# lazytiger/pbrt-rs

Hardware: AMD Instinct MI355X
Metric: Mrays/s (higher is better)
Workload: dtype f32

## Files before the change

pbrt-rs_amd/csrc/render.hip:

```cpp
#include <hip/hip_runtime.h>
#include "abi_guard.h"

#include <algorithm>
#include <chrono>
#include <cstdio>
#include <cstdlib>
#include <cstring>
#include <string>
#include <thread>
#include <vector>

#include "scene.h"
#include "trace.h"
#include "wavefront.h"

using namespace pb;

extern "C" int pbrt_hip_render_device(PbrtHipScene* s, const PbrtCamera* camera, const PbrtRenderParams* params,
                                      float* d_film, PbrtRenderStats* stats) try {
    if (!s || !camera || !params || !d_film) return PBRT_HIP_ERR_INVALID;
    PB_ENTER(s->ctx);
    HIP_TRY(s->ctx, hipSetDevice(s->ctx->device));
    return wavefront_render(s, *camera, *params, d_film, stats);
}
// ... 622 lines not shown
        if (stats) *stats = local;
        return PBRT_HIP_OK;
    }
    const int n_pix = (int)origins.size() * kTile * kTile;
    int64_t valid_pixels = 0;
    for (const int2& o : origins)
        valid_pixels += (int64_t)(std::min(o.x + kTile, rp.x1) - o.x) * (std::min(o.y + kTile, rp.y1) - o.y);
    if (li_mode) valid_pixels = li->n;
    if (export_mode) rp.spp_per_pass = rp.spp;
    int spp_pass = rp.spp_per_pass > 0 ? rp.spp_per_pass : 0;
    if (spp_pass == 0) {
        size_t free_b = 0, total_b = 0;
        HIP_TRY(ctx, hipMemGetInfo(&free_b, &total_b));
        for (const auto& b : ctx->block_cache)
            if (!b.in_use) free_b += b.bytes;
        const int64_t per_path = 400 + (rp.integrator != PBRT_INTEGRATOR_PATH ? 24 + 48ll * std::max(1, rp.max_depth) : 0);
        const int64_t target_paths = std::max<int64_t>(1ll << 20, std::min<int64_t>(1ll << 28, (int64_t)(free_b / 2) / per_path));
        spp_pass = (int)std::max<int64_t>(1, std::min<int64_t>(rp.spp, target_paths / n_pix));
    }
    spp_pass = std::min(spp_pass, rp.spp);
    if (export_mode && spp_pass != rp.spp) return invalid("camera rays: too many samples for one pass");
    const size_t N = (size_t)n_pix * spp_pass;
    if (N * 4 >= (1ull << 32)) return invalid("too many concurrent paths for 32-bit queue entries; lower spp_per_pass");

    DevBuf buf(ctx);
    bool ok = true;
    PathState ps;
    ps.n_paths = N;
    ps.two_level = s->d.bvh.instanced ? 1 : 0;
    ps.ray = buf.alloc<float4>(N * 6, &ok);
    ps.hit = buf.alloc<float4>(N * 6, &ok);
    ps.rng = buf.alloc<uint64_t>(N, &ok);
    ps.L = buf.alloc<float4>(N, &ok);
    ps.beta = buf.alloc<float4>(N, &ok);
    ps.nee_a = buf.alloc<float4>(N, &ok);
    ps.nee_f = buf.alloc<float4>(N, &ok);
    ps.nee_b = buf.alloc<float4>(N, &ok);
    ps.nee_light = buf.alloc<int>(N, &ok);
    ps.pfilm = buf.alloc<float2>(N, &ok);
    Queues q[2];
    for (int k = 0; k < 2; ++k) {
        q[k].trace = buf.alloc<uint32_t>(N * 3, &ok);
        q[k].shade = buf.alloc<uint32_t>(N, &ok);
        q[k].counts64 = buf.alloc<unsigned long long>(2, &ok);
        q[k].keys = nullptr;
        for (int a = 0; a < 3; ++a) {
            const float lo = s->d.bvh.root_min[a], hi = s->d.bvh.root_max[a];
            q[k].key_lo[a] = lo;
            q[k].key_inv[a] = hi > lo ? 1.0f / (hi - lo) : 0.0f;
        }
    }
    if (rp.ray_order < 0 || rp.ray_order > 1) return invalid("ray_order must be 0 (Morton order from the second bounce on) or 1 (queue order)");
    const bool sort_rays = rp.ray_order == 0 && rp.integrator == PBRT_INTEGRATOR_PATH;
    constexpr int sort_from = 2;
// ... 3 lines not shown
    if (sort_rays) {
        sort_keys[0] = buf.alloc<uint32_t>(N * 3, &ok);
        sort_keys[1] = buf.alloc<uint32_t>(N * 3, &ok);
        sort_vals = buf.alloc<uint32_t>(N * 3, &ok);
        if (pb::sort_pairs_u32(st, nullptr, &sort_tmp_bytes, sort_keys[0], sort_keys[1], sort_vals, sort_vals, N * 3, kSortKeyBits) != 0)
            return invalid("rocPRIM radix sort: size query failed");
        sort_tmp = buf.alloc<char>(sort_tmp_bytes, &ok);
    }
    const bool use_wide = s->has_wide && ctx->count_traversal != 1 && ctx->traversal == PBRT_TRAVERSAL_AUTO;
    const bool stackless = ctx->traversal == PBRT_TRAVERSAL_STACKLESS;
    if (stackless && !stackless_applies(s)) return PBRT_HIP_ERR_INVALID;
    uint32_t* special_list = use_wide ? buf.alloc<uint32_t>(N * 3, &ok) : nullptr;
    if (rp.shade_order < 0 || rp.shade_order > 2) return invalid("shade_order must be 0 (queue order), 1 (by material inside blocks) or 2 (sorted queue)");
    const bool sort_shade = rp.shade_order == 2 && rp.integrator == PBRT_INTEGRATOR_PATH;
    const bool bin_shade = rp.shade_order == 1 && rp.integrator == PBRT_INTEGRATOR_PATH;
    uint32_t *shade_keys[2] = {nullptr, nullptr}, *shade_sorted = nullptr;
    void* shade_tmp = nullptr;
    size_t shade_tmp_bytes = 0;
    if (sort_shade) {
        shade_keys[0] = buf.alloc<uint32_t>(N, &ok);
        shade_keys[1] = buf.alloc<uint32_t>(N, &ok);
        shade_sorted = buf.alloc<uint32_t>(N, &ok);
        if (pb::sort_pairs_u32(st, nullptr, &shade_tmp_bytes, shade_keys[0], shade_keys[1], shade_sorted, shade_sorted, N, 3) != 0)
            return invalid("rocPRIM radix sort: size query failed");
        shade_tmp = buf.alloc<char>(shade_tmp_bytes, &ok);
    }
    DirectState ds{};
    std::vector<int> prefix(s->d.n_lights + 1, 0);
    for (int i = 0; i < s->d.n_lights; ++i)
        prefix[i + 1] = prefix[i] + (tabulated ? round_count(s->light_samples[i]) : s->light_samples[i]);
    SamplerParams smp{};
    smp.kind = rp.sampler;
    smp.n_dims = rp.sampler_dims;
    smp.nx = rp.sampler_x;
    smp.ny = rp.sampler_y;
    smp.jitter = rp.sampler_jitter;
    ps.samp = buf.alloc<int>(N, &ok);
    if (rp.sampler == PBRT_SAMPLER_HALTON) {
// ... 285 lines not shown
            if (direct)
{
                dim3 sg((n_shade + 255) / 256), sb(256);
                if (rp.integrator == PBRT_INTEGRATOR_DIRECT && s->glossy)
                    hipLaunchKernelGGL((k_shade_direct<PBRT_INTEGRATOR_DIRECT, true>), sg, sb, 0, st, sc, ps, ds, q[cur], q[nxt], pp, tiles, n_shade);
                else if (rp.integrator == PBRT_INTEGRATOR_DIRECT)
                    hipLaunchKernelGGL((k_shade_direct<PBRT_INTEGRATOR_DIRECT, false>), sg, sb, 0, st, sc, ps, ds, q[cur], q[nxt], pp, tiles, n_shade);
                else if (rp.integrator == PBRT_INTEGRATOR_WHITTED && s->glossy)
                    hipLaunchKernelGGL((k_shade_direct<PBRT_INTEGRATOR_WHITTED, true>), sg, sb, 0, st, sc, ps, ds, q[cur], q[nxt], pp, tiles, n_shade);
                else if (rp.integrator == PBRT_INTEGRATOR_WHITTED)
                    hipLaunchKernelGGL((k_shade_direct<PBRT_INTEGRATOR_WHITTED, false>), sg, sb, 0, st, sc, ps, ds, q[cur], q[nxt], pp, tiles, n_shade);
                else
                    hipLaunchKernelGGL((k_shade_direct<PBRT_INTEGRATOR_AO, false>), sg, sb, 0, st, sc, ps, ds, q[cur], q[nxt], pp, tiles, n_shade);
            }
            else {
                Queues qin = q[cur];
                if (sort_shade && wavefront >= 1 && n_shade >= (1u << 10)) {
                    hipLaunchKernelGGL(k_shade_sort_keys, dim3((n_shade + 255) / 256), dim3(256), 0, st, sc, ps, q[cur].shade, n_shade,
                                       pp.max_depth, shade_keys[0]);
                    size_t tb = shade_tmp_bytes;
                    if (pb::sort_pairs_u32(st, shade_tmp, &tb, shade_keys[0], shade_keys[1], q[cur].shade, shade_sorted, n_shade, 3) != 0 &&
                        rc == PBRT_HIP_OK) {
                        ctx->last_error = "rocPRIM radix sort failed";
                        rc = PBRT_HIP_ERR_DEVICE;
                    }
                    qin.shade = shade_sorted;
                }
                const dim3 sg((n_shade + 255) / 256), sb(256);
                if (bin_shade && wavefront >= 1 && s->glossy)
                    hipLaunchKernelGGL((k_shade<true, true>), sg, sb, 0, st, sc, ps, qin, q[nxt], pp, tiles, n_shade);
                else if (bin_shade && wavefront >= 1)
                    hipLaunchKernelGGL((k_shade<true, false>), sg, sb, 0, st, sc, ps, qin, q[nxt], pp, tiles, n_shade);
                else if (s->glossy)
                    hipLaunchKernelGGL((k_shade<false, true>), sg, sb, 0, st, sc, ps, qin, q[nxt], pp, tiles, n_shade);
                else
                    hipLaunchKernelGGL((k_shade<false, false>), sg, sb, 0, st, sc, ps, qin, q[nxt], pp, tiles, n_shade);
            }
            RENDER_TRY(hipGetLastError());
            RENDER_TRY(hipMemcpyAsync(ctx->h_counts, q[nxt].counts64, sizeof(counts), hipMemcpyDeviceToHost, st));
            RENDER_TRY(hipEventRecord(ctx->ev_sync, st));
            if (rc == PBRT_HIP_OK) {
                hipError_t qe;
                const auto spin_start = std::chrono::steady_clock::now();
                uint32_t polls = 0;
                while ((qe = hipEventQuery(ctx->ev_sync)) == hipErrorNotReady) {
                    if ((++polls & 0xfffu) == 0) {
                        const double waited = std::chrono::duration<double>(std::chrono::steady_clock::now() - spin_start).count();
                        if (waited > ctx->wavefront_deadline_s) {
                            ctx->last_error = "a wavefront did not finish within the deadline (hung kernel?)";
                            ctx->lost = true;
                            rc = PBRT_HIP_ERR_DEVICE;
                            break;
                        }
                        if (waited > 0.05) std::this_thread::yield();
                    }
                }
                if (rc == PBRT_HIP_OK) RENDER_TRY(qe);
            }
            counts[0] = ctx->h_counts[0];
            counts[1] = ctx->h_counts[1];
            if (n_trace > 0 && rc == PBRT_HIP_OK) {
                float ms = 0.0f;
                RENDER_TRY(hipEventElapsedTime(&ms, e_t0, e_t1));
                local.trace_ms += ms;
                local.trace_launches += 1;
                if (ctx->trace_log)
                    std::fprintf(stderr, "[pbrt_hip] k_trace: %u rays %.3f ms (%.0f Mrays/s)\n", n_trace, ms, n_trace / ms * 1e-3);
                ctx->trace_ms += ms;
                ctx->trace_launches += 1;
            }
            {
                uint64_t n_rays = counts[0] & 0xffffffffull, n_shadow = counts[0] >> 32;
                local.rays_closest += n_rays - n_shadow;
                local.rays_shadow += n_shadow;
                counts[0] = n_rays;
            }
            (void)first;
            first = false;
            wavefront += 1;
            cur = nxt;
        }
        if (li_mode) {
// ... 56 lines not shown
```

pbrt-rs_amd/csrc/wf_direct.h:

```cpp
#pragma once
#include "wf_path.h"

namespace pb {

struct DirectState {
    int* stage;
    float4* ld_acc;
    float4* frames;
    int light_strategy;
    int mode;
    int ao_samples;
    int ao_cos_sample;
};

#ifndef PB_DIRECT_WAVES
#define PB_DIRECT_WAVES 2
#endif
template <int MODE, bool GLOSSY>
__global__ void __launch_bounds__(256, (GLOSSY && MODE == PBRT_INTEGRATOR_DIRECT) ? 1 : PB_DIRECT_WAVES) k_shade_direct(ShadeConsts sc, PathState ps, DirectState ds, Queues qin,
                                                        Queues qout, PassParams pp, TileList tiles, uint32_t n_in) {
    uint32_t i = blockIdx.x * blockDim.x + threadIdx.x;
    bool active = i < n_in;
    uint32_t p = active ? qin.shade[i] : 0u;
    bool emit_cont = false, emit_mis = false, emit_shadow = false, mis_bool = false;
// ... 187 lines not shown
                    pick_pdf = 1.0f / nl;
                }
                float ul0, ul1, us0, us1;
                if (sample_all && tabulated && !fallback) {
                    int k = stage - sc.light_sample_prefix[light_num];
                    int first = (sm.arr & 0x7fff) - 2 * sc.n_lights + 2 * light_num;
                    samp_array_2d(pp, sm, first, k, &ul0, &ul1);
                    samp_array_2d(pp, sm, first + 1, k, &us0, &us1);
                } else {
                    samp_2d(pp, sm, &ul0, &ul1);
                    samp_2d(pp, sm, &us0, &us1);
                }
                int nee_flags;
                if (GLOSSY) {
                    NsBsdf nsb = ns_bsdf(sc.materials[sf.material]);
                    nee_flags = estimate_direct_emit(sc, ps, p, sf, fr, nsb.n > 0, nsb, light_num, ul0, ul1, us0, us1, pick_pdf, T);
                } else {
                    bool matte = (mat.type == PBRT_MAT_MATTE) && !is_black(kd);
                    nee_flags = estimate_direct_emit(sc, ps, p, sf, fr, matte, MatteBsdf{kd}, light_num, ul0, ul1, us0, us1, pick_pdf, T);
                }
                stage += 1;
                if (nee_flags) {
                    flags |= nee_flags & 0xff;
                    emit_shadow = (nee_flags & PF_NEE_SHADOW) != 0;
                    emit_mis = (nee_flags & PF_NEE_MIS) != 0;
                    mis_bool = (nee_flags & NEE_MIS_BOOL) != 0;
                    break;
                }
                close_light_if_done(stage);
                continue;
            }
            bool branched = false;
            if ((stage == total || stage == total + 1) && depth + 1 < pp.max_depth && mode != PBRT_INTEGRATOR_AO) {
                if (!surface_ready) load_surface();
// ... 67 lines not shown
```

pbrt-rs_amd/csrc/wf_lights.h:

```cpp
#pragma once
#include "wf_microfacet.h"

namespace pb {

PB_DEV V3 sphere_through(V3 v) {
    return V3{1.0f * v.x + 0.0f * v.y + 0.0f * v.z, 0.0f * v.x + 1.0f * v.y + 0.0f * v.z, 0.0f * v.x + 0.0f * v.y + 1.0f * v.z};
}
PB_DEV float sphere_area(float radius) { return (360.0f * (kPi / 180.0f)) * radius * (radius - (-radius)); }
PB_DEV void sphere_light_sample(float cx, float cy, float cz, float radius, const Surf& sf, float u0, float u1, V3* p_o,
                                V3* err_o, V3* n_o, float* pdf_o) {
    V3 pc = V3{1.0f * 0.0f + 0.0f * 0.0f + 0.0f * 0.0f + cx, 0.0f * 0.0f + 1.0f * 0.0f + 0.0f * 0.0f + cy,
               0.0f * 0.0f + 0.0f * 0.0f + 1.0f * 0.0f + cz};
    V3 p_origin = offset_ray_origin(sf.p, sf.p_error, sf.n, pc - sf.p);
    if (len2(p_origin - pc) <= radius * radius) {
        float z = 1.0f - 2.0f * u0;
        float rr = __builtin_sqrtf(fmaxr(1.0f - z * z, 0.0f));
        float sp, cp;
        det_sincos(2.0f * kPi * u1, &sp, &cp);
        V3 obj = V3{rr * cp, rr * sp, z} * radius;
        V3 n = normalize(sphere_through(obj));
        obj = obj * (radius / length(obj));
        V3 oe = vabs(obj) * kGamma5;
        const float g3 = kGamma3;
        V3 p = V3{1.0f * obj.x + 0.0f * obj.y + 0.0f * obj.z + cx, 0.0f * obj.x + 1.0f * obj.y + 0.0f * obj.z + cy,
// ... 216 lines not shown
    for (int j = 0; j < n; ++j) sum += func[j];
    float avg = sum / (float)(128 * n);
    float min_contrib = avg > 0.0f ? 0.001f * avg : 1.0f;
    for (int j = 0; j < n; ++j) func[j] = fmaxr(func[j], min_contrib);
    cdf[0] = 0.0f;
    for (int j = 1; j < n + 1; ++j) cdf[j] = cdf[j - 1] + func[j - 1] / (float)n;
    float func_int = cdf[n];
    if (func_int == 0.0f) {
        for (int j = 1; j < n + 1; ++j) cdf[j] = (float)j / (float)n;
    } else {
        for (int j = 1; j < n + 1; ++j) cdf[j] /= func_int;
    }
    func[2 * n + 1] = func_int;
}

template <class Bsdf>
PB_DEV int estimate_direct_emit(const ShadeConsts& sc, const PathState& ps, uint32_t p, const Surf& sf, const Frame& fr,
                                bool nonspecular, const Bsdf& bsdf, int light_num, float ul0, float ul1, float us0, float us1,
                                float pick_pdf, V3 beta) {
    if (!nonspecular) return 0;
    V3 wo = sf.wo;
    DevLight lt = sc.lights[light_num];
    V3 wi, li, p1, p1_err, p1_n;
    float light_pdf;
    light_sample_li(sc, sf, lt, ul0, ul1, &wi, &light_pdf, &li, &p1, &p1_err, &p1_n);
    int nee_flags = 0;
    V3 A = V3{0.0f, 0.0f, 0.0f};
    if (light_pdf > 0.0f && !is_black(li)) {
        V3 f;
        float scattering_pdf;
        bsdf_f_pdf(bsdf, fr, wo, wi, &f, &scattering_pdf);
        f = f * absdot(wi, fr.ns);
        if (!is_black(f)) {
            V3 origin = offset_ray_origin(sf.p, sf.p_error, sf.n, p1 - sf.p);
            V3 target = offset_ray_origin(p1, p1_err, p1_n, origin - p1);
            V3 d = target - origin;
            store_ray(ps, p, RS_SHADOW, origin, d, 1.0f - kShadowEpsilon);
            if (lt.delta) {
                A = mulv(li, f) / light_pdf;
            } else {
                float weight = power_heuristic1(light_pdf, scattering_pdf);
                A = mulv(li, f) * weight / light_pdf;
            }
            nee_flags |= PF_NEE_SHADOW;
        }
    }
    V3 wi2;
    float spdf = 0.0f;
    bool ok = false;
    V3 f2 = V3{0.0f, 0.0f, 0.0f};
    if (!lt.delta) f2 = bsdf_sample_f(bsdf, fr, wo, us0, us1, &wi2, &spdf, &ok);
    if (ok) f2 = f2 * absdot(wi2, fr.ns);
// ... 40 lines not shown
            if (ph < 0.0f) ph = ph + 2.0f * kPi;
            float st = det_sin(theta);
            if (st == 0.0f) {
                lpdf = 0.0f;
            } else {
                int iu = (int)(ph * kInv2Pi * 2.0f);
                iu = iu < 0 ? 0 : (iu > 1 ? 1 : iu);
                int iv = (int)(theta * kInvPi * 2.0f);
                iv = iv < 0 ? 0 : (iv > 1 ? 1 : iv);
                lpdf = sc.env_cond_func[iv][iu] / sc.env_marg_int / (2.0f * kPi * kPi * st);
            }
        }
        if (lpdf != 0.0f) {
            float weight = power_heuristic1(spdf, lpdf);
            V3 o2 = offset_ray_origin(sf.p, sf.p_error, sf.n, wi2);
            store_ray(ps, p, RS_MIS, o2, wi2, kInf);
            ps.nee_f[p] = make_float4(f2.x, f2.y, f2.z, weight);
            nee_flags |= PF_NEE_MIS;
            if (sc.mis_bool && lt.type != PBRT_LIGHT_DIFFUSE_AREA) nee_flags |= NEE_MIS_BOOL;
        }
    }
    if (nee_flags) {
        ps.nee_a[p] = make_float4(A.x, A.y, A.z, pick_pdf);
        ps.nee_b[p] = make_float4(beta.x, beta.y, beta.z, spdf);
        ps.nee_light[p] = light_num;
    }
    return nee_flags;
}

PB_DEV V3 estimate_direct_resolve(const ShadeConsts& sc, const PathState& ps, uint32_t p, int flags, float* pick_pdf,
                                  V3* beta_at_vertex) {
    float4 na = ps.nee_a[p], nf = ps.nee_f[p], nb = ps.nee_b[p];
    int light_id = ps.nee_light[p];
    V3 ld = V3{0.0f, 0.0f, 0.0f};
    if (flags & PF_NEE_SHADOW) {
        bool occluded = ps.hit[hit_index(ps, p, RS_SHADOW)].x != 0.0f;
        if (!occluded) ld = ld + V3{na.x, na.y, na.z};
    }
    if (flags & PF_NEE_MIS) {
        int hslot = __float_as_int(ps.hit[hit_index(ps, p, RS_MIS)].x);
        DevLight lt = sc.lights[light_id];
        V3 li = V3{0.0f, 0.0f, 0.0f};
        if (hslot >= 0) {
            int hl = lt.type == PBRT_LIGHT_DIFFUSE_AREA ? (__float_as_int(sc.bvh.tris[3 * (size_t)hslot + 2].w) & kPrimLightMask) - 1 : -2;
            if (hl == light_id) {
                float4 r0 = ps.ray[ray_index(ps, p, RS_MIS)], r1 = ps.ray[ray_index(ps, p, RS_MIS) + 1];
                V3 wi = V3{r0.w, r1.x, r1.y};
                float4 hb = ps.hit[hit_index(ps, p, RS_MIS)];
                V3 n = tri_interaction_normal(sc.bvh, hslot, hb.y, hb.z, hb.w);
                if (lt.two_sided || dot(n, -wi) > 0.0f) li = V3{lt.L[0], lt.L[1], lt.L[2]};
            }
        } else if (lt.type == PBRT_LIGHT_INFINITE) {
            if (lt.slot >= 0) {
                float4 r0 = ps.ray[ray_index(ps, p, RS_MIS)], r1 = ps.ray[ray_index(ps, p, RS_MIS) + 1];
                li = env_le(sc.env_maps[lt.slot], V3{r0.w, r1.x, r1.y});
            } else {
                li = V3{lt.L[0], lt.L[1], lt.L[2]};
            }
        }
        if (!is_black(li)) {
            V3 f = V3{nf.x, nf.y, nf.z};
            ld = ld + mulv(li, f) * nf.w / nb.w;
        }
    }
    *pick_pdf = na.w;
    *beta_at_vertex = V3{nb.x, nb.y, nb.z};
    return ld;
}

// ... 49 lines not shown
```

pbrt-rs_amd/csrc/wf_path.h:

```cpp
#pragma once
#include "wf_lights.h"

namespace pb {

PB_DEV uint32_t shade_key(const ShadeConsts& sc, const PathState& ps, uint32_t p, int max_depth) {
    int fb = __float_as_int(ps.beta[p].w);
    uint32_t key = 0;
    if ((fb & PF_ALIVE) && (fb >> 8) < max_depth) {
        const size_t hb = hit_index(ps, p, RS_CONT);
        int slot = __float_as_int(ps.hit[hb].x), inst = hit_instance(ps, hb);
        if (slot >= 0) {
            int mat = __float_as_int(sc.bvh.tris[3 * (size_t)slot + 2].z);
            if (sc.bvh.instanced && inst >= 0) {
                int over = __float_as_int(sc.bvh.instances[7 * (size_t)inst + 6].x);
                if (over >= 0) mat = over;
            }
            key = 1u + (uint32_t)sc.materials[mat].type;
        }
    }
    return key;
}
__global__ void k_shade_sort_keys(ShadeConsts sc, PathState ps, const uint32_t* __restrict__ shade_queue, uint32_t n, int max_depth,
                                  uint32_t* __restrict__ keys) {
    uint32_t i = blockIdx.x * blockDim.x + threadIdx.x;
    if (i >= n) return;
    keys[i] = shade_key(sc, ps, shade_queue[i], max_depth);
}

constexpr int shade_keys(bool glossy) { return glossy ? 8 : 6; }
template <int KEYS>
struct ShadeBins {
    uint32_t count[4][KEYS];
    uint32_t path[256];
};

#ifndef PB_SHADE_WAVES
#define PB_SHADE_WAVES 3
#endif
template <bool BIN, bool GLOSSY>
__global__ void __launch_bounds__(256, PB_SHADE_WAVES) k_shade(ShadeConsts sc, PathState ps, Queues qin, Queues qout, PassParams pp,
                                                 TileList tiles, uint32_t n_in) {
    constexpr int kShadeKeys = shade_keys(GLOSSY);
    uint32_t i = blockIdx.x * blockDim.x + threadIdx.x;
    bool active = i < n_in;
    uint32_t p = active ? qin.shade[i] : 0u;
    if (BIN) {
        __shared__ ShadeBins<kShadeKeys> bins;
        const int lane = threadIdx.x & 63, wave = threadIdx.x >> 6;
        const uint32_t key = active ? shade_key(sc, ps, p, pp.max_depth) : (uint32_t)(kShadeKeys - 1);
        uint32_t rank = 0;
#pragma unroll
        for (int k = 0; k < kShadeKeys; ++k) {
            const unsigned long long m = __ballot(key == (uint32_t)k);
            if (key == (uint32_t)k) rank = lane_prefix(m);
            if (lane == 0) bins.count[wave][k] = (uint32_t)__popcll(m);
        }
        __syncthreads();
        uint32_t before = 0;
        for (int k = 0; k < kShadeKeys; ++k)
            for (int w = 0; w < 4; ++w)
                before += ((uint32_t)k < key || ((uint32_t)k == key && w < wave)) ? bins.count[w][k] : 0u;
        bins.path[before + rank] = p;
        uint32_t n_active = 0;
        for (int k = 0; k < kShadeKeys - 1; ++k)
            for (int w = 0; w < 4; ++w) n_active += bins.count[w][k];
        __syncthreads();
        p = bins.path[threadIdx.x];
        active = threadIdx.x < n_active;
    }
    bool emit_cont = false, emit_mis = false, emit_shadow = false, mis_bool = false;

    uint32_t cell = 0;
    if (active) {
        float4 Lq = ps.L[p], bq = ps.beta[p];
        V3 L = V3{Lq.x, Lq.y, Lq.z};
        float eta_scale = Lq.w;
        V3 beta = V3{bq.x, bq.y, bq.z};
        int fb = __float_as_int(bq.w);
        int flags = fb & 0xff, bounces = fb >> 8;
        size_t rbase = ray_index(ps, p, RS_CONT), hbase = hit_index(ps, p, RS_CONT);

        if (flags & (PF_NEE_SHADOW | PF_NEE_MIS)) {
            float pick_pdf;
            V3 beta_v;
            V3 ld = estimate_direct_resolve(sc, ps, p, flags, &pick_pdf, &beta_v);
            ld = ld / pick_pdf;
            L = L + mulv(beta_v, ld);
            flags &= ~(PF_NEE_SHADOW | PF_NEE_MIS);
        }

        if (flags & PF_ALIVE) {
            flags &= ~PF_ALIVE;
            float4 r0 = ps.ray[rbase], r1 = ps.ray[rbase + 1];
            V3 rd = V3{r0.w, r1.x, r1.y};
            float4 h0 = ps.hit[hbase];
            int hslot = __float_as_int(h0.x);
            bool found = hslot >= 0;
            Surf sf;
            if (found) {
                sf = surface_from_hit(sc.bvh, hslot, hit_instance(ps, hbase), h0.y, h0.z, h0.w, rd);
// ... 3 lines not shown
                if (found) {
                    L = L + mulv(beta, surface_le(sc, sf, -rd));
                } else {
                    for (int k = 0; k < sc.n_infinite; ++k) {
                        DevLight lt = sc.lights[sc.infinite_ids[k]];
                        V3 le = lt.slot >= 0 ? env_le(sc.env_maps[lt.slot], rd) : V3{lt.L[0], lt.L[1], lt.L[2]};
                        L = L + mulv(beta, le);
                    }
                }
            }
            if (found && bounces < pp.max_depth) {
                DevMaterial mat = sc.materials[sf.material];
                Samp sm = path_sampler(ps, pp, tiles, p);
                if (mat.type == PBRT_MAT_NONE) {
                    V3 o = offset_ray_origin(sf.p, sf.p_error, sf.n, rd);
                    store_ray(ps, p, RS_CONT, o, rd, kInf);
                    flags |= PF_ALIVE;
                    emit_cont = true;
                } else {
                    Frame fr = make_frame(sf);
                    V3 kd = V3{mat.kd[0], mat.kd[1], mat.kd[2]};
                    V3 kt = V3{mat.kt[0], mat.kt[1], mat.kt[2]};
                    V3 wo = -rd;
                    bool has_lobe;
                    bool nonspecular;
                    NsBsdf nsb;
                    if (GLOSSY) {
                        nsb = ns_bsdf(mat);
                        nonspecular = nsb.n > 0;
                        if (mat.type == PBRT_MAT_GLASS) has_lobe = !(is_black(kd) && is_black(kt));
                        else if (mat.type == PBRT_MAT_MIRROR) has_lobe = !is_black(kd);
// ... 2 lines not shown
                        if (mat.type == PBRT_MAT_GLASS) has_lobe = !(is_black(kd) && is_black(kt));
                        else has_lobe = !is_black(kd);
                        nonspecular = (mat.type == PBRT_MAT_MATTE) && has_lobe;
                    }

                    if (nonspecular && sc.n_lights > 0) {
                        float u_pick = samp_1d(pp, sm);
                        DevDistribution1D distrib = light_distribution_lookup(sc, sf.p);
                        int light_num = find_interval_cdf(distrib.cdf, distrib.n + 1, u_pick);
                        float pick_pdf = distrib.func_int > 0.0f ? distrib.func[light_num] / (distrib.func_int * (float)distrib.n)
                                                                 : 0.0f;
                        if (pick_pdf != 0.0f) {
                            float ul0, ul1, us0, us1;
                            samp_2d(pp, sm, &ul0, &ul1);
                            samp_2d(pp, sm, &us0, &us1);
                            int nee_flags = GLOSSY ? estimate_direct_emit(sc, ps, p, sf, fr, true, nsb, light_num, ul0, ul1, us0,
                                                                          us1, pick_pdf, beta)
                                                   : estimate_direct_emit(sc, ps, p, sf, fr, true, MatteBsdf{kd}, light_num, ul0, ul1,
                                                                          us0, us1, pick_pdf, beta);
                            flags |= nee_flags & 0xff;
                            emit_shadow = (nee_flags & PF_NEE_SHADOW) != 0;
                            emit_mis = (nee_flags & PF_NEE_MIS) != 0;
                            mis_bool = (nee_flags & NEE_MIS_BOOL) != 0;
                        }
                    }

                    float u0 = 0.0f, u1 = 0.0f;
                    samp_2d(pp, sm, &u0, &u1);
                    V3 wi = V3{0.0f, 0.0f, 0.0f}, f = V3{0.0f, 0.0f, 0.0f};
                    float pdf = 0.0f;
                    bool sampled_specular = false, sampled_transmission = false;
                    if (has_lobe) {
                        if (GLOSSY && nonspecular) {
// ... 20 lines not shown
                        beta = mulv(beta, f * (absdot(wi, fr.ns) / pdf));
                        flags = (flags & ~PF_SPECULAR_BOUNCE) | (sampled_specular ? PF_SPECULAR_BOUNCE : 0);
                        if (sampled_specular && sampled_transmission) {
                            float eta = mat.eta;
                            eta_scale *= (dot(wo, sf.n) > 0.0f) ? (eta * eta) : 1.0f / (eta * eta);
                        }
                        V3 o = offset_ray_origin(sf.p, sf.p_error, sf.n, wi);
                        bool alive = true;
                        V3 rr_beta = beta * eta_scale;
                        if (max_comp(rr_beta) < pp.rr_threshold && bounces > 3) {
                            float qq = fmaxr(0.05f, 1.0f - max_comp(rr_beta));
                            if (samp_1d(pp, sm) < qq) alive = false;
                            else beta = beta / (1.0f - qq);
                        }
                        if (alive) {
                            store_ray(ps, p, RS_CONT, o, wi, kInf);
                            flags |= PF_ALIVE;
                            emit_cont = true;
                            bounces += 1;
                        }
                    }
                }
                samp_store(ps, p, sm);
            }
        }
        ps.L[p] = make_float4(L.x, L.y, L.z, eta_scale);
        ps.beta[p] = make_float4(beta.x, beta.y, beta.z, __int_as_float((bounces << 8) | flags));
    }

    __shared__ BlockAppend sh;
    const bool again = emit_cont || emit_mis || emit_shadow;
    block_append(sh, qout, p, emit_cont, emit_mis, emit_shadow, again, cell, mis_bool);
}

}
```

pbrt-rs_amd/csrc/wf_state.h:

```cpp
#pragma once
#include <hip/hip_runtime.h>

#include "scene.h"
#include "trace.h"
#include "trace_persistent.h"
#include "trace_wide.h"
#include "trace_stackless.h"

namespace pb {

constexpr int kTile = 16;
enum PathFlags : int {
    PF_SPECULAR_BOUNCE = 1,
    PF_ALIVE = 2,
    PF_NEE_SHADOW = 4,
    PF_NEE_MIS = 8,
    PF_VALID = 16,
};
enum RaySlot : int { RS_CONT = 0, RS_MIS = 1, RS_SHADOW = 2 };
constexpr uint32_t RS_MIS_BOOL = 3;
constexpr int NEE_MIS_BOOL = 0x100;

struct PathState {
    float4* ray;
    float4* hit;
    size_t n_paths;
    uint64_t* rng;
    float4* L;
    float4* beta;
    float4* nee_a;
    float4* nee_f;
    float4* nee_b;
    int* nee_light;
    float2* pfilm;
    int* samp;
    int two_level;
};
PB_DEV int hit_instance(const PathState& ps, size_t hit_base) { return ps.two_level ? __float_as_int(ps.hit[hit_base + 1].x) : -1; }

#ifndef PB_RAY_PATH_MAJOR
#define PB_RAY_PATH_MAJOR 0
#endif
#ifndef PB_HIT_PATH_MAJOR
#define PB_HIT_PATH_MAJOR 0
#endif
PB_DEV size_t ray_index(const PathState& ps, uint32_t p, int slot) {
    return PB_RAY_PATH_MAJOR ? ((size_t)p * 3 + slot) * 2 : ((size_t)slot * ps.n_paths + p) * 2;
}
PB_DEV size_t hit_index(const PathState& ps, uint32_t p, int slot) {
    return PB_HIT_PATH_MAJOR ? ((size_t)p * 3 + slot) * 2 : ((size_t)slot * ps.n_paths + p) * 2;
}

struct SamplerParams {
    int kind;
    int n_dims;
    int nx, ny, jitter;
    int n_arrays;
    int off2;
    int n_elems;
    float* tables;
    const int2* arrays;
    int h_scale[2], h_exp[2];
    int h_stride, array_end_dim;
    unsigned int h_minv[2];
    const uint16_t* perms;
// ... 61 lines not shown
    return (int64_t)(y - pp.sb_y0) * pp.sb_w + (x - pp.sb_x0);
}
PB_DEV uint64_t sample_sequence(const PassParams& pp, int x, int y, int s) {
    return pp.seed ^ (uint64_t)(pixel_number(pp, x, y) * (int64_t)pp.spp + s);
}

struct BlockAppend {
    uint32_t wave_rays[16];
    uint32_t wave_shadow[16];
    uint32_t wave_paths[16];
    uint32_t base_rays, base_paths;
};
PB_DEV uint32_t lane_prefix(unsigned long long mask) {
    return __builtin_amdgcn_mbcnt_hi((uint32_t)(mask >> 32), __builtin_amdgcn_mbcnt_lo((uint32_t)mask, 0));
}
PB_DEV void block_append(BlockAppend& sh, const Queues& q, uint32_t p, bool cont, bool mis, bool shadow, bool again,
                         uint32_t cell = 0, bool mis_bool = false) {
    const int lane = threadIdx.x & 63, wave = threadIdx.x >> 6, n_waves = (blockDim.x + 63) >> 6;
    unsigned long long mc = __ballot(cont), mm = __ballot(mis), ms = __ballot(shadow), ma = __ballot(again);
    uint32_t wc = (uint32_t)__popcll(mc), wm = (uint32_t)__popcll(mm), ws = (uint32_t)__popcll(ms);
    if (lane == 0) {
        sh.wave_rays[wave] = wc + wm + ws;
        sh.wave_shadow[wave] = ws;
        sh.wave_paths[wave] = (uint32_t)__popcll(ma);
    }
    __syncthreads();
    if (threadIdx.x == 0) {
        uint32_t tr = 0, tsd = 0, tp = 0;
        for (int w = 0; w < n_waves; ++w) {
            uint32_t r = sh.wave_rays[w], pth = sh.wave_paths[w];
            sh.wave_rays[w] = tr;
            sh.wave_paths[w] = tp;
            tr += r;
            tsd += sh.wave_shadow[w];
            tp += pth;
        }
        unsigned long long old = 0;
        if (tr) old = atomicAdd(&q.counts64[0], (unsigned long long)tr | ((unsigned long long)tsd << 32));
        sh.base_rays = (uint32_t)old;
        sh.base_paths = tp ? (uint32_t)atomicAdd(&q.counts64[1], (unsigned long long)tp) : 0u;
    }
    __syncthreads();
    uint32_t rbase = sh.base_rays + sh.wave_rays[wave];
    uint32_t ic = rbase + lane_prefix(mc), im = rbase + wc + lane_prefix(mm), is = rbase + wc + wm + lane_prefix(ms);
    if (cont) q.trace[ic] = p * 4u + RS_CONT;
    if (mis) q.trace[im] = p * 4u + (mis_bool ? RS_MIS_BOOL : (uint32_t)RS_MIS);
    if (shadow) q.trace[is] = p * 4u + RS_SHADOW;
    if (q.keys) {
        if (cont) q.keys[ic] = cell;
        if (mis) q.keys[im] = mis_bool ? (cell | (1u << (kSortKeyBits - 1))) : cell;
        if (shadow) q.keys[is] = cell | (1u << (kSortKeyBits - 1));
    }
    if (again) q.shade[sh.base_paths + sh.wave_paths[wave] + lane_prefix(ma)] = p;
}

PB_DEV void store_ray(const PathState& ps, uint32_t p, int slot, V3 o, V3 d, float tmax) {
    size_t i = ray_index(ps, p, slot);
    ps.ray[i] = make_float4(o.x, o.y, o.z, d.x);
    ps.ray[i + 1] = make_float4(d.y, d.z, tmax, 0.0f);
}

struct DevCamera {
    float c2w[16], r2c[16];
    float lens_radius, focal_distance, shutter_open, shutter_close;
    int kind;
};
PB_DEV V3 xform_point(const float* m, V3 p) {
    float xp = m[0] * p.x + m[1] * p.y + m[2] * p.z + m[3];
    float yp = m[4] * p.x + m[5] * p.y + m[6] * p.z + m[7];
    float zp = m[8] * p.x + m[9] * p.y + m[10] * p.z + m[11];
    float wp = m[12] * p.x + m[13] * p.y + m[14] * p.z + m[15];
    if (wp == 1.0f) return V3{xp, yp, zp};
    return V3{xp, yp, zp} / wp;
}
PB_DEV V3 xform_vector(const float* m, V3 v) {
// ... 11 lines not shown
```

Measured before the change: 2903.

## Compact per-path ray and NEE records into output queue order via LDS staging

The path shading kernel now stages its outgoing rays and NEE records in shared memory and writes them to double-buffered arrays indexed by the new shade-queue slot, so the next bounce reads ray, hit and NEE data contiguously instead of scattered by path id. Shade sorting now sorts positions rather than path ids. The pass-size heuristic is retuned for the path integrator to account for the extra buffers. The cost is more device memory, about 24 KB of shared memory per block (which may lower occupancy), and an extra copy through LDS.

```diff
diff --git a/pbrt-rs_amd/csrc/render.hip b/pbrt-rs_amd/csrc/render.hip
--- a/pbrt-rs_amd/csrc/render.hip
+++ b/pbrt-rs_amd/csrc/render.hip
@@ -660,8 +660,9 @@
         HIP_TRY(ctx, hipMemGetInfo(&free_b, &total_b));
         for (const auto& b : ctx->block_cache)
             if (!b.in_use) free_b += b.bytes;
-        const int64_t per_path = 400 + (rp.integrator != PBRT_INTEGRATOR_PATH ? 24 + 48ll * std::max(1, rp.max_depth) : 0);
-        const int64_t target_paths = std::max<int64_t>(1ll << 20, std::min<int64_t>(1ll << 28, (int64_t)(free_b / 2) / per_path));
+        const int64_t per_path = rp.integrator == PBRT_INTEGRATOR_PATH ? 550 : 400 + 24 + 48ll * std::max(1, rp.max_depth);
+        const size_t share = rp.integrator == PBRT_INTEGRATOR_PATH ? free_b / 3 * 2 : free_b / 2;
+        const int64_t target_paths = std::max<int64_t>(1ll << 20, std::min<int64_t>(1ll << 28, (int64_t)share / per_path));
         spp_pass = (int)std::max<int64_t>(1, std::min<int64_t>(rp.spp, target_paths / n_pix));
     }
     spp_pass = std::min(spp_pass, rp.spp);
@@ -684,6 +685,11 @@
     ps.nee_b = buf.alloc<float4>(N, &ok);
     ps.nee_light = buf.alloc<int>(N, &ok);
     ps.pfilm = buf.alloc<float2>(N, &ok);
+    ps.ray_next = direct ? ps.ray : buf.alloc<float4>(N * 6, &ok);
+    ps.nee_a_next = direct ? ps.nee_a : buf.alloc<float4>(N, &ok);
+    ps.nee_f_next = direct ? ps.nee_f : buf.alloc<float4>(N, &ok);
+    ps.nee_b_next = direct ? ps.nee_b : buf.alloc<float4>(N, &ok);
+    ps.nee_light_next = direct ? ps.nee_light : buf.alloc<int>(N, &ok);
     Queues q[2];
     for (int k = 0; k < 2; ++k) {
         q[k].trace = buf.alloc<uint32_t>(N * 3, &ok);
@@ -717,14 +723,15 @@
     if (rp.shade_order < 0 || rp.shade_order > 2) return invalid("shade_order must be 0 (queue order), 1 (by material inside blocks) or 2 (sorted queue)");
     const bool sort_shade = rp.shade_order == 2 && rp.integrator == PBRT_INTEGRATOR_PATH;
     const bool bin_shade = rp.shade_order == 1 && rp.integrator == PBRT_INTEGRATOR_PATH;
-    uint32_t *shade_keys[2] = {nullptr, nullptr}, *shade_sorted = nullptr;
+    uint32_t *shade_keys[2] = {nullptr, nullptr}, *shade_positions = nullptr, *shade_sorted = nullptr;
     void* shade_tmp = nullptr;
     size_t shade_tmp_bytes = 0;
     if (sort_shade) {
         shade_keys[0] = buf.alloc<uint32_t>(N, &ok);
         shade_keys[1] = buf.alloc<uint32_t>(N, &ok);
+        shade_positions = buf.alloc<uint32_t>(N, &ok);
         shade_sorted = buf.alloc<uint32_t>(N, &ok);
-        if (pb::sort_pairs_u32(st, nullptr, &shade_tmp_bytes, shade_keys[0], shade_keys[1], shade_sorted, shade_sorted, N, 3) != 0)
+        if (pb::sort_pairs_u32(st, nullptr, &shade_tmp_bytes, shade_keys[0], shade_keys[1], shade_positions, shade_sorted, N, 3) != 0)
             return invalid("rocPRIM radix sort: size query failed");
         shade_tmp = buf.alloc<char>(shade_tmp_bytes, &ok);
     }
@@ -1040,27 +1047,33 @@
                     hipLaunchKernelGGL((k_shade_direct<PBRT_INTEGRATOR_AO, false>), sg, sb, 0, st, sc, ps, ds, q[cur], q[nxt], pp, tiles, n_shade);
             }
             else {
-                Queues qin = q[cur];
+                const Queues qin = q[cur];
+                const uint32_t* order = nullptr;
                 if (sort_shade && wavefront >= 1 && n_shade >= (1u << 10)) {
                     hipLaunchKernelGGL(k_shade_sort_keys, dim3((n_shade + 255) / 256), dim3(256), 0, st, sc, ps, q[cur].shade, n_shade,
-                                       pp.max_depth, shade_keys[0]);
+                                       pp.max_depth, shade_keys[0], shade_positions);
                     size_t tb = shade_tmp_bytes;
-                    if (pb::sort_pairs_u32(st, shade_tmp, &tb, shade_keys[0], shade_keys[1], q[cur].shade, shade_sorted, n_shade, 3) != 0 &&
+                    if (pb::sort_pairs_u32(st, shade_tmp, &tb, shade_keys[0], shade_keys[1], shade_positions, shade_sorted, n_shade, 3) != 0 &&
                         rc == PBRT_HIP_OK) {
                         ctx->last_error = "rocPRIM radix sort failed";
                         rc = PBRT_HIP_ERR_DEVICE;
                     }
-                    qin.shade = shade_sorted;
+                    order = shade_sorted;
                 }
                 const dim3 sg((n_shade + 255) / 256), sb(256);
                 if (bin_shade && wavefront >= 1 && s->glossy)
-                    hipLaunchKernelGGL((k_shade<true, true>), sg, sb, 0, st, sc, ps, qin, q[nxt], pp, tiles, n_shade);
+                    hipLaunchKernelGGL((k_shade<true, true>), sg, sb, 0, st, sc, ps, qin, q[nxt], pp, tiles, n_shade, order);
                 else if (bin_shade && wavefront >= 1)
-                    hipLaunchKernelGGL((k_shade<true, false>), sg, sb, 0, st, sc, ps, qin, q[nxt], pp, tiles, n_shade);
+                    hipLaunchKernelGGL((k_shade<true, false>), sg, sb, 0, st, sc, ps, qin, q[nxt], pp, tiles, n_shade, order);
                 else if (s->glossy)
-                    hipLaunchKernelGGL((k_shade<false, true>), sg, sb, 0, st, sc, ps, qin, q[nxt], pp, tiles, n_shade);
+                    hipLaunchKernelGGL((k_shade<false, true>), sg, sb, 0, st, sc, ps, qin, q[nxt], pp, tiles, n_shade, order);
                 else
-                    hipLaunchKernelGGL((k_shade<false, false>), sg, sb, 0, st, sc, ps, qin, q[nxt], pp, tiles, n_shade);
+                    hipLaunchKernelGGL((k_shade<false, false>), sg, sb, 0, st, sc, ps, qin, q[nxt], pp, tiles, n_shade, order);
+                std::swap(ps.ray, ps.ray_next);
+                std::swap(ps.nee_a, ps.nee_a_next);
+                std::swap(ps.nee_f, ps.nee_f_next);
+                std::swap(ps.nee_b, ps.nee_b_next);
+                std::swap(ps.nee_light, ps.nee_light_next);
             }
             RENDER_TRY(hipGetLastError());
             RENDER_TRY(hipMemcpyAsync(ctx->h_counts, q[nxt].counts64, sizeof(counts), hipMemcpyDeviceToHost, st));
@@ -1091,7 +1104,8 @@
                 local.trace_ms += ms;
                 local.trace_launches += 1;
                 if (ctx->trace_log)
-                    std::fprintf(stderr, "[pbrt_hip] k_trace: %u rays %.3f ms (%.0f Mrays/s)\n", n_trace, ms, n_trace / ms * 1e-3);
+                    std::fprintf(stderr, "[pbrt_hip] k_trace: %u rays %.3f ms (%.0f Mrays/s), k_shade: %u paths\n", n_trace, ms, n_trace / ms * 1e-3,
+                                 n_shade);
                 ctx->trace_ms += ms;
                 ctx->trace_launches += 1;
             }
diff --git a/pbrt-rs_amd/csrc/wf_direct.h b/pbrt-rs_amd/csrc/wf_direct.h
--- a/pbrt-rs_amd/csrc/wf_direct.h
+++ b/pbrt-rs_amd/csrc/wf_direct.h
@@ -225,10 +225,10 @@
                 int nee_flags;
                 if (GLOSSY) {
                     NsBsdf nsb = ns_bsdf(sc.materials[sf.material]);
-                    nee_flags = estimate_direct_emit(sc, ps, p, sf, fr, nsb.n > 0, nsb, light_num, ul0, ul1, us0, us1, pick_pdf, T);
+                    nee_flags = estimate_direct_emit(sc, RecordSink{ps, p}, sf, fr, nsb.n > 0, nsb, light_num, ul0, ul1, us0, us1, pick_pdf, T);
                 } else {
                     bool matte = (mat.type == PBRT_MAT_MATTE) && !is_black(kd);
-                    nee_flags = estimate_direct_emit(sc, ps, p, sf, fr, matte, MatteBsdf{kd}, light_num, ul0, ul1, us0, us1, pick_pdf, T);
+                    nee_flags = estimate_direct_emit(sc, RecordSink{ps, p}, sf, fr, matte, MatteBsdf{kd}, light_num, ul0, ul1, us0, us1, pick_pdf, T);
                 }
                 stage += 1;
                 if (nee_flags) {
diff --git a/pbrt-rs_amd/csrc/wf_lights.h b/pbrt-rs_amd/csrc/wf_lights.h
--- a/pbrt-rs_amd/csrc/wf_lights.h
+++ b/pbrt-rs_amd/csrc/wf_lights.h
@@ -254,8 +254,8 @@
     func[2 * n + 1] = func_int;
 }
 
-template <class Bsdf>
-PB_DEV int estimate_direct_emit(const ShadeConsts& sc, const PathState& ps, uint32_t p, const Surf& sf, const Frame& fr,
+template <class Bsdf, class Sink>
+PB_DEV int estimate_direct_emit(const ShadeConsts& sc, const Sink& out, const Surf& sf, const Frame& fr,
                                 bool nonspecular, const Bsdf& bsdf, int light_num, float ul0, float ul1, float us0, float us1,
                                 float pick_pdf, V3 beta) {
     if (!nonspecular) return 0;
@@ -275,7 +275,7 @@
             V3 origin = offset_ray_origin(sf.p, sf.p_error, sf.n, p1 - sf.p);
             V3 target = offset_ray_origin(p1, p1_err, p1_n, origin - p1);
             V3 d = target - origin;
-            store_ray(ps, p, RS_SHADOW, origin, d, 1.0f - kShadowEpsilon);
+            out.ray(RS_SHADOW, origin, d, 1.0f - kShadowEpsilon);
             if (lt.delta) {
                 A = mulv(li, f) / light_pdf;
             } else {
@@ -346,45 +346,45 @@
         if (lpdf != 0.0f) {
             float weight = power_heuristic1(spdf, lpdf);
             V3 o2 = offset_ray_origin(sf.p, sf.p_error, sf.n, wi2);
-            store_ray(ps, p, RS_MIS, o2, wi2, kInf);
-            ps.nee_f[p] = make_float4(f2.x, f2.y, f2.z, weight);
+            out.ray(RS_MIS, o2, wi2, kInf);
+            out.nee_f(make_float4(f2.x, f2.y, f2.z, weight));
             nee_flags |= PF_NEE_MIS;
             if (sc.mis_bool && lt.type != PBRT_LIGHT_DIFFUSE_AREA) nee_flags |= NEE_MIS_BOOL;
         }
     }
     if (nee_flags) {
-        ps.nee_a[p] = make_float4(A.x, A.y, A.z, pick_pdf);
-        ps.nee_b[p] = make_float4(beta.x, beta.y, beta.z, spdf);
-        ps.nee_light[p] = light_num;
+        out.nee_a(make_float4(A.x, A.y, A.z, pick_pdf));
+        out.nee_b(make_float4(beta.x, beta.y, beta.z, spdf));
+        out.nee_light(light_num);
     }
     return nee_flags;
 }
 
-PB_DEV V3 estimate_direct_resolve(const ShadeConsts& sc, const PathState& ps, uint32_t p, int flags, float* pick_pdf,
+PB_DEV V3 estimate_direct_resolve(const ShadeConsts& sc, const PathState& ps, uint32_t rec, int flags, float* pick_pdf,
                                   V3* beta_at_vertex) {
-    float4 na = ps.nee_a[p], nf = ps.nee_f[p], nb = ps.nee_b[p];
-    int light_id = ps.nee_light[p];
+    float4 na = ps.nee_a[rec], nf = ps.nee_f[rec], nb = ps.nee_b[rec];
+    int light_id = ps.nee_light[rec];
     V3 ld = V3{0.0f, 0.0f, 0.0f};
     if (flags & PF_NEE_SHADOW) {
-        bool occluded = ps.hit[hit_index(ps, p, RS_SHADOW)].x != 0.0f;
+        bool occluded = ps.hit[hit_index(ps, rec, RS_SHADOW)].x != 0.0f;
         if (!occluded) ld = ld + V3{na.x, na.y, na.z};
     }
     if (flags & PF_NEE_MIS) {
-        int hslot = __float_as_int(ps.hit[hit_index(ps, p, RS_MIS)].x);
+        int hslot = __float_as_int(ps.hit[hit_index(ps, rec, RS_MIS)].x);
         DevLight lt = sc.lights[light_id];
         V3 li = V3{0.0f, 0.0f, 0.0f};
         if (hslot >= 0) {
             int hl = lt.type == PBRT_LIGHT_DIFFUSE_AREA ? (__float_as_int(sc.bvh.tris[3 * (size_t)hslot + 2].w) & kPrimLightMask) - 1 : -2;
             if (hl == light_id) {
-                float4 r0 = ps.ray[ray_index(ps, p, RS_MIS)], r1 = ps.ray[ray_index(ps, p, RS_MIS) + 1];
+                float4 r0 = ps.ray[ray_index(ps, rec, RS_MIS)], r1 = ps.ray[ray_index(ps, rec, RS_MIS) + 1];
                 V3 wi = V3{r0.w, r1.x, r1.y};
-                float4 hb = ps.hit[hit_index(ps, p, RS_MIS)];
+                float4 hb = ps.hit[hit_index(ps, rec, RS_MIS)];
                 V3 n = tri_interaction_normal(sc.bvh, hslot, hb.y, hb.z, hb.w);
                 if (lt.two_sided || dot(n, -wi) > 0.0f) li = V3{lt.L[0], lt.L[1], lt.L[2]};
             }
         } else if (lt.type == PBRT_LIGHT_INFINITE) {
             if (lt.slot >= 0) {
-                float4 r0 = ps.ray[ray_index(ps, p, RS_MIS)], r1 = ps.ray[ray_index(ps, p, RS_MIS) + 1];
+                float4 r0 = ps.ray[ray_index(ps, rec, RS_MIS)], r1 = ps.ray[ray_index(ps, rec, RS_MIS) + 1];
                 li = env_le(sc.env_maps[lt.slot], V3{r0.w, r1.x, r1.y});
             } else {
                 li = V3{lt.L[0], lt.L[1], lt.L[2]};
diff --git a/pbrt-rs_amd/csrc/wf_path.h b/pbrt-rs_amd/csrc/wf_path.h
--- a/pbrt-rs_amd/csrc/wf_path.h
+++ b/pbrt-rs_amd/csrc/wf_path.h
@@ -3,11 +3,11 @@
 
 namespace pb {
 
-PB_DEV uint32_t shade_key(const ShadeConsts& sc, const PathState& ps, uint32_t p, int max_depth) {
+PB_DEV uint32_t shade_key(const ShadeConsts& sc, const PathState& ps, uint32_t p, uint32_t rec, int max_depth) {
     int fb = __float_as_int(ps.beta[p].w);
     uint32_t key = 0;
     if ((fb & PF_ALIVE) && (fb >> 8) < max_depth) {
-        const size_t hb = hit_index(ps, p, RS_CONT);
+        const size_t hb = hit_index(ps, rec, RS_CONT);
         int slot = __float_as_int(ps.hit[hb].x), inst = hit_instance(ps, hb);
         if (slot >= 0) {
             int mat = __float_as_int(sc.bvh.tris[3 * (size_t)slot + 2].z);
@@ -21,10 +21,11 @@
     return key;
 }
 __global__ void k_shade_sort_keys(ShadeConsts sc, PathState ps, const uint32_t* __restrict__ shade_queue, uint32_t n, int max_depth,
-                                  uint32_t* __restrict__ keys) {
+                                  uint32_t* __restrict__ keys, uint32_t* __restrict__ positions) {
     uint32_t i = blockIdx.x * blockDim.x + threadIdx.x;
     if (i >= n) return;
-    keys[i] = shade_key(sc, ps, shade_queue[i], max_depth);
+    keys[i] = shade_key(sc, ps, shade_queue[i], i, max_depth);
+    positions[i] = i;
 }
 
 constexpr int shade_keys(bool glossy) { return glossy ? 8 : 6; }
@@ -32,6 +33,7 @@
 struct ShadeBins {
     uint32_t count[4][KEYS];
     uint32_t path[256];
+    uint32_t rec[256];
 };
 
 #ifndef PB_SHADE_WAVES
@@ -39,15 +41,18 @@
 #endif
 template <bool BIN, bool GLOSSY>
 __global__ void __launch_bounds__(256, PB_SHADE_WAVES) k_shade(ShadeConsts sc, PathState ps, Queues qin, Queues qout, PassParams pp,
-                                                 TileList tiles, uint32_t n_in) {
+                                                 TileList tiles, uint32_t n_in, const uint32_t* __restrict__ order) {
     constexpr int kShadeKeys = shade_keys(GLOSSY);
     uint32_t i = blockIdx.x * blockDim.x + threadIdx.x;
     bool active = i < n_in;
-    uint32_t p = active ? qin.shade[i] : 0u;
+    uint32_t rec = (active && order) ? order[i] : i;
+    uint32_t p = active ? qin.shade[rec] : 0u;
+    __shared__ StagedRecords staged;
+    const StageSink stage{staged};
     if (BIN) {
         __shared__ ShadeBins<kShadeKeys> bins;
         const int lane = threadIdx.x & 63, wave = threadIdx.x >> 6;
-        const uint32_t key = active ? shade_key(sc, ps, p, pp.max_depth) : (uint32_t)(kShadeKeys - 1);
+        const uint32_t key = active ? shade_key(sc, ps, p, rec, pp.max_depth) : (uint32_t)(kShadeKeys - 1);
         uint32_t rank = 0;
 #pragma unroll
         for (int k = 0; k < kShadeKeys; ++k) {
@@ -61,11 +66,13 @@
             for (int w = 0; w < 4; ++w)
                 before += ((uint32_t)k < key || ((uint32_t)k == key && w < wave)) ? bins.count[w][k] : 0u;
         bins.path[before + rank] = p;
+        bins.rec[before + rank] = rec;
         uint32_t n_active = 0;
         for (int k = 0; k < kShadeKeys - 1; ++k)
             for (int w = 0; w < 4; ++w) n_active += bins.count[w][k];
         __syncthreads();
         p = bins.path[threadIdx.x];
+        rec = bins.rec[threadIdx.x];
         active = threadIdx.x < n_active;
     }
     bool emit_cont = false, emit_mis = false, emit_shadow = false, mis_bool = false;
@@ -78,12 +85,12 @@
         V3 beta = V3{bq.x, bq.y, bq.z};
         int fb = __float_as_int(bq.w);
         int flags = fb & 0xff, bounces = fb >> 8;
-        size_t rbase = ray_index(ps, p, RS_CONT), hbase = hit_index(ps, p, RS_CONT);
+        size_t rbase = ray_index(ps, rec, RS_CONT), hbase = hit_index(ps, rec, RS_CONT);
 
         if (flags & (PF_NEE_SHADOW | PF_NEE_MIS)) {
             float pick_pdf;
             V3 beta_v;
-            V3 ld = estimate_direct_resolve(sc, ps, p, flags, &pick_pdf, &beta_v);
+            V3 ld = estimate_direct_resolve(sc, ps, rec, flags, &pick_pdf, &beta_v);
             ld = ld / pick_pdf;
             L = L + mulv(beta_v, ld);
             flags &= ~(PF_NEE_SHADOW | PF_NEE_MIS);
@@ -117,7 +124,7 @@
                 Samp sm = path_sampler(ps, pp, tiles, p);
                 if (mat.type == PBRT_MAT_NONE) {
                     V3 o = offset_ray_origin(sf.p, sf.p_error, sf.n, rd);
-                    store_ray(ps, p, RS_CONT, o, rd, kInf);
+                    stage.ray(RS_CONT, o, rd, kInf);
                     flags |= PF_ALIVE;
                     emit_cont = true;
                 } else {
@@ -150,9 +157,9 @@
                             float ul0, ul1, us0, us1;
                             samp_2d(pp, sm, &ul0, &ul1);
                             samp_2d(pp, sm, &us0, &us1);
-                            int nee_flags = GLOSSY ? estimate_direct_emit(sc, ps, p, sf, fr, true, nsb, light_num, ul0, ul1, us0,
+                            int nee_flags = GLOSSY ? estimate_direct_emit(sc, stage, sf, fr, true, nsb, light_num, ul0, ul1, us0,
                                                                           us1, pick_pdf, beta)
-                                                   : estimate_direct_emit(sc, ps, p, sf, fr, true, MatteBsdf{kd}, light_num, ul0, ul1,
+                                                   : estimate_direct_emit(sc, stage, sf, fr, true, MatteBsdf{kd}, light_num, ul0, ul1,
                                                                           us0, us1, pick_pdf, beta);
                             flags |= nee_flags & 0xff;
                             emit_shadow = (nee_flags & PF_NEE_SHADOW) != 0;
@@ -203,7 +210,7 @@
                             else beta = beta / (1.0f - qq);
                         }
                         if (alive) {
-                            store_ray(ps, p, RS_CONT, o, wi, kInf);
+                            stage.ray(RS_CONT, o, wi, kInf);
                             flags |= PF_ALIVE;
                             emit_cont = true;
                             bounces += 1;
@@ -219,7 +226,9 @@
 
     __shared__ BlockAppend sh;
     const bool again = emit_cont || emit_mis || emit_shadow;
-    block_append(sh, qout, p, emit_cont, emit_mis, emit_shadow, again, cell, mis_bool);
-}
-
-}
+    const AppendSlots slots = block_reserve(sh, qout, emit_cont, emit_mis, emit_shadow, again);
+    stage.flush(ps, slots.shade, emit_cont, emit_mis, emit_shadow);
+    block_write(qout, slots, p, slots.shade, emit_cont, emit_mis, emit_shadow, again, cell, mis_bool);
+}
+
+}
diff --git a/pbrt-rs_amd/csrc/wf_state.h b/pbrt-rs_amd/csrc/wf_state.h
--- a/pbrt-rs_amd/csrc/wf_state.h
+++ b/pbrt-rs_amd/csrc/wf_state.h
@@ -34,6 +34,9 @@
     int* nee_light;
     float2* pfilm;
     int* samp;
+    float4* ray_next;
+    float4 *nee_a_next, *nee_f_next, *nee_b_next;
+    int* nee_light_next;
     int two_level;
 };
 PB_DEV int hit_instance(const PathState& ps, size_t hit_base) { return ps.two_level ? __float_as_int(ps.hit[hit_base + 1].x) : -1; }
@@ -44,11 +47,11 @@
 #ifndef PB_HIT_PATH_MAJOR
 #define PB_HIT_PATH_MAJOR 0
 #endif
-PB_DEV size_t ray_index(const PathState& ps, uint32_t p, int slot) {
-    return PB_RAY_PATH_MAJOR ? ((size_t)p * 3 + slot) * 2 : ((size_t)slot * ps.n_paths + p) * 2;
-}
-PB_DEV size_t hit_index(const PathState& ps, uint32_t p, int slot) {
-    return PB_HIT_PATH_MAJOR ? ((size_t)p * 3 + slot) * 2 : ((size_t)slot * ps.n_paths + p) * 2;
+PB_DEV size_t ray_index(const PathState& ps, uint32_t j, int slot) {
+    return PB_RAY_PATH_MAJOR ? ((size_t)j * 3 + slot) * 2 : ((size_t)slot * ps.n_paths + j) * 2;
+}
+PB_DEV size_t hit_index(const PathState& ps, uint32_t j, int slot) {
+    return PB_HIT_PATH_MAJOR ? ((size_t)j * 3 + slot) * 2 : ((size_t)slot * ps.n_paths + j) * 2;
 }
 
 struct SamplerParams {
@@ -140,8 +143,10 @@
 PB_DEV uint32_t lane_prefix(unsigned long long mask) {
     return __builtin_amdgcn_mbcnt_hi((uint32_t)(mask >> 32), __builtin_amdgcn_mbcnt_lo((uint32_t)mask, 0));
 }
-PB_DEV void block_append(BlockAppend& sh, const Queues& q, uint32_t p, bool cont, bool mis, bool shadow, bool again,
-                         uint32_t cell = 0, bool mis_bool = false) {
+struct AppendSlots {
+    uint32_t cont, mis, shadow, shade;
+};
+PB_DEV AppendSlots block_reserve(BlockAppend& sh, const Queues& q, bool cont, bool mis, bool shadow, bool again) {
     const int lane = threadIdx.x & 63, wave = threadIdx.x >> 6, n_waves = (blockDim.x + 63) >> 6;
     unsigned long long mc = __ballot(cont), mm = __ballot(mis), ms = __ballot(shadow), ma = __ballot(again);
     uint32_t wc = (uint32_t)__popcll(mc), wm = (uint32_t)__popcll(mm), ws = (uint32_t)__popcll(ms);
@@ -168,23 +173,86 @@
     }
     __syncthreads();
     uint32_t rbase = sh.base_rays + sh.wave_rays[wave];
-    uint32_t ic = rbase + lane_prefix(mc), im = rbase + wc + lane_prefix(mm), is = rbase + wc + wm + lane_prefix(ms);
-    if (cont) q.trace[ic] = p * 4u + RS_CONT;
-    if (mis) q.trace[im] = p * 4u + (mis_bool ? RS_MIS_BOOL : (uint32_t)RS_MIS);
-    if (shadow) q.trace[is] = p * 4u + RS_SHADOW;
+    AppendSlots a;
+    a.cont = rbase + lane_prefix(mc);
+    a.mis = rbase + wc + lane_prefix(mm);
+    a.shadow = rbase + wc + wm + lane_prefix(ms);
+    a.shade = sh.base_paths + sh.wave_paths[wave] + lane_prefix(ma);
+    return a;
+}
+PB_DEV void block_write(const Queues& q, const AppendSlots& a, uint32_t p, uint32_t rec, bool cont, bool mis, bool shadow, bool again,
+                        uint32_t cell, bool mis_bool) {
+    if (cont) q.trace[a.cont] = rec * 4u + RS_CONT;
+    if (mis) q.trace[a.mis] = rec * 4u + (mis_bool ? RS_MIS_BOOL : (uint32_t)RS_MIS);
+    if (shadow) q.trace[a.shadow] = rec * 4u + RS_SHADOW;
     if (q.keys) {
-        if (cont) q.keys[ic] = cell;
-        if (mis) q.keys[im] = mis_bool ? (cell | (1u << (kSortKeyBits - 1))) : cell;
-        if (shadow) q.keys[is] = cell | (1u << (kSortKeyBits - 1));
-    }
-    if (again) q.shade[sh.base_paths + sh.wave_paths[wave] + lane_prefix(ma)] = p;
-}
-
-PB_DEV void store_ray(const PathState& ps, uint32_t p, int slot, V3 o, V3 d, float tmax) {
-    size_t i = ray_index(ps, p, slot);
+        if (cont) q.keys[a.cont] = cell;
+        if (mis) q.keys[a.mis] = mis_bool ? (cell | (1u << (kSortKeyBits - 1))) : cell;
+        if (shadow) q.keys[a.shadow] = cell | (1u << (kSortKeyBits - 1));
+    }
+    if (again) q.shade[a.shade] = p;
+}
+PB_DEV void block_append(BlockAppend& sh, const Queues& q, uint32_t p, bool cont, bool mis, bool shadow, bool again,
+                         uint32_t cell = 0, bool mis_bool = false) {
+    const AppendSlots a = block_reserve(sh, q, cont, mis, shadow, again);
+    block_write(q, a, p, p, cont, mis, shadow, again, cell, mis_bool);
+}
+
+PB_DEV void store_ray(const PathState& ps, uint32_t j, int slot, V3 o, V3 d, float tmax) {
+    size_t i = ray_index(ps, j, slot);
     ps.ray[i] = make_float4(o.x, o.y, o.z, d.x);
     ps.ray[i + 1] = make_float4(d.y, d.z, tmax, 0.0f);
 }
+
+struct RecordSink {
+    const PathState& ps;
+    uint32_t rec;
+    PB_DEV void ray(int slot, V3 o, V3 d, float tmax) const { store_ray(ps, rec, slot, o, d, tmax); }
+    PB_DEV void nee_a(float4 v) const { ps.nee_a[rec] = v; }
+    PB_DEV void nee_f(float4 v) const { ps.nee_f[rec] = v; }
+    PB_DEV void nee_b(float4 v) const { ps.nee_b[rec] = v; }
+    PB_DEV void nee_light(int v) const { ps.nee_light[rec] = v; }
+};
+struct StagedRecords {
+    float4 ray[3][2][256];
+    float4 nee_a[256], nee_f[256], nee_b[256];
+    int nee_light[256];
+};
+struct StageSink {
+    StagedRecords& st;
+    PB_DEV void ray(int slot, V3 o, V3 d, float tmax) const {
+        st.ray[slot][0][threadIdx.x] = make_float4(o.x, o.y, o.z, d.x);
+        st.ray[slot][1][threadIdx.x] = make_float4(d.y, d.z, tmax, 0.0f);
+    }
+    PB_DEV void nee_a(float4 v) const { st.nee_a[threadIdx.x] = v; }
+    PB_DEV void nee_f(float4 v) const { st.nee_f[threadIdx.x] = v; }
+    PB_DEV void nee_b(float4 v) const { st.nee_b[threadIdx.x] = v; }
+    PB_DEV void nee_light(int v) const { st.nee_light[threadIdx.x] = v; }
+    PB_DEV void flush(const PathState& ps, uint32_t j, bool cont, bool mis, bool shadow) const {
+        const uint32_t t = threadIdx.x;
+        if (cont) {
+            size_t i = ray_index(ps, j, RS_CONT);
+            ps.ray_next[i] = st.ray[RS_CONT][0][t];
+            ps.ray_next[i + 1] = st.ray[RS_CONT][1][t];
+        }
+        if (mis) {
+            size_t i = ray_index(ps, j, RS_MIS);
+            ps.ray_next[i] = st.ray[RS_MIS][0][t];
+            ps.ray_next[i + 1] = st.ray[RS_MIS][1][t];
+            ps.nee_f_next[j] = st.nee_f[t];
+        }
+        if (shadow) {
+            size_t i = ray_index(ps, j, RS_SHADOW);
+            ps.ray_next[i] = st.ray[RS_SHADOW][0][t];
+            ps.ray_next[i + 1] = st.ray[RS_SHADOW][1][t];
+        }
+        if (mis || shadow) {
+            ps.nee_a_next[j] = st.nee_a[t];
+            ps.nee_b_next[j] = st.nee_b[t];
+            ps.nee_light_next[j] = st.nee_light[t];
+        }
+    }
+};
 
 struct DevCamera {
     float c2w[16], r2c[16];
```

Result: faster. 3005, median of 6 (+3.5%).
